# NeuralRevenant/RASSEngine

Hardware: NVIDIA B200
Metric: exact top-10 QPS @10M x 1024 (cosine, ids identical to the fp64 CPU oracle) (higher is better)
Workload: dtype bf16 scan (fp32 accumulate) + fp64 rerank

## Files before the change

rassengine_b200/csrc/common.cuh:

```cuda
#pragma once
#include <cuda_runtime.h>
#include <cuda_bf16.h>
#include <stdint.h>
#include <stdio.h>
#include <string>
#include <vector>

#include "../../include/rass_b200.h"

#define RASS_WARPS_PER_CTA 8
#define RASS_MAX_K 128
#define RASS_CAND_MAX 2048
#define RASS_GROUP_Q 64
#define RASS_QPAD 256
#define RASS_STREAM_SEG 64
static inline int rass_tc_seg(int k) { return k > 32 ? 512 : 256; }
__host__ __device__ constexpr int rass_tc_keep(int seg) { return seg == 512 ? 128 : seg / 8; }
#define RASS_EXACT_NQ 4
#define RASS_FINISH_THREADS 1024

struct RowMap {
  int64_t base;
  int32_t g, G, blk_log2;
};
#define RASS_SHARD_BLOCK_LOG2 10
__host__ __device__ inline int64_t row_local_to_global(const RowMap& m, int64_t local) {
  if (m.G <= 1) return m.base + local;
  const int64_t b = local >> m.blk_log2, in = local & ((int64_t(1) << m.blk_log2) - 1);
  return m.base + (((b * m.G + m.g) << m.blk_log2) | in);
}
__host__ __device__ inline int64_t row_global_to_local(const RowMap& m, int64_t global) {
  const int64_t r = global - m.base;
  if (r < 0) return -1;
  if (m.G <= 1) return r;
  const int64_t b = r >> m.blk_log2;
  if ((int32_t)(b % m.G) != m.g) return -1;
  return ((b / m.G) << m.blk_log2) | (r & ((int64_t(1) << m.blk_log2) - 1));
}

#define HYB_TILE 4096
#define HYB_TABLE_MIN_DF 512

struct TextSegment {
  int field = 0;
  int64_t n_post = 0, n_uniq = 0;
  int32_t* uterm = nullptr;
  int64_t* uptr = nullptr;
  int32_t* doc = nullptr;
  uint16_t* tf = nullptr;
};

struct Bm25State {
  bool built = false;
  int64_t V = 0, N = 0, nnz = 0;
  int F = 1;
  std::vector<uint8_t> term_field_host;
  int64_t* indptr = nullptr;
  int32_t* doc = nullptr;
  uint16_t* tf = nullptr;
  float* xq = nullptr;
  uint8_t* norm = nullptr;
  float* inv_dev = nullptr;
  int n_tiles = 0;
  uint32_t* tile_off = nullptr;
  std::vector<int32_t> table_row_host;
  unsigned char* qt_host = nullptr;
  unsigned char* qt_dev = nullptr;
  size_t qt_cap = 0, qt_q_cap = 0, qt_bytes = 0;
  uint32_t* hyb_gthr = nullptr;
  uint32_t* vocab_blob = nullptr;
  int64_t* vocab_off = nullptr;
  int64_t vocab_V = 0;
  int32_t* fz_terms = nullptr;
  int32_t* fz_edits = nullptr;
  int* fz_n = nullptr;
  float avgdl = 0.f;
  int64_t doc_count = 0;
  std::vector<int64_t> indptr_host;
  std::vector<float> idf_host;
  std::vector<float> xmin_host, xmax_host;
  bool force_ordered = false;
  bool maxscore = false;
  int* sel_fallback = nullptr;
  std::vector<TextSegment> pending;
  uint32_t* doclen_dev = nullptr;
  uint32_t* gen_dev = nullptr;
  bool has_rewrite = false;
  int doclen_F = 0;
  int64_t doclen_stride = 0;
  std::vector<int64_t> field_vocab;
  std::vector<int64_t> field_last_row;
  bool contiguous_fields = true;
  std::vector<int64_t> field_doc_count, field_sum_ttf;
  std::vector<uint8_t> field_omit_norms;
  int64_t pending_V = 0;
  void* scratch = nullptr;
  size_t scratch_bytes = 0;
};

struct StoreScalars {
  float rho_x;
  float max_xnorm;
  float rho_x8;
};

struct SearchScalars {
  int flagged_n;
  int max_cand;
  int n_certified;
  int finish_done;
  int tile_ctr[2];
};

struct SearchWs {
  SearchScalars* scal = nullptr;
  int q_cap = 0;
  float* q_raw = nullptr;
  float* q_hat = nullptr;
  __nv_bfloat16* q16 = nullptr;
  double* q_norm = nullptr;
  float* q_rho = nullptr;
  int8_t* q8 = nullptr;
  float* q8_scale = nullptr;
  float* q_rho8 = nullptr;
  uint32_t* q_gthr = nullptr;
  size_t pool_entries = 0;
  size_t pool_alloc_entries = 0;
  float* pool_key = nullptr;
  uint32_t* pool_row = nullptr;
  size_t pool_segs = 0;
  size_t pool_alloc_segs = 0;
  float* pool_thr = nullptr;
  int* pool_cnt = nullptr;
  int* flagged = nullptr;
  int* flagged_host = nullptr;
  void* tmap_q = nullptr;
  void* tmap_q2 = nullptr;
  const void* tmap_qbase = nullptr;
  const void* tmap_q2base = nullptr;
  void* tmap_q8 = nullptr;
  const void* tmap_q8base = nullptr;
};

struct VmArray {
  void* base = nullptr;
  size_t reserved = 0, mapped = 0, chunk = 0;
  int device = 0;
  std::vector<unsigned long long> handles;
};
bool vm_available();
bool vm_reserve(VmArray* a, int device, size_t max_bytes, size_t chunk_hint);
int vm_grow(VmArray* a, size_t bytes);
void vm_free(VmArray* a);

struct rass_engine {
  int dim = 0, dim_pad = 0, metric = 0, device = 0;
  uint32_t flags = 0;
  int num_sms = 0;
  int path = RASS_PATH_AUTO;
  int64_t cap = 0, n_rows = 0, n_live = 0;
  RowMap rmap = {0, 0, 1, RASS_SHARD_BLOCK_LOG2};
  struct ShardSet* shards = nullptr;
  float* x32 = nullptr;
  __nv_bfloat16* x16 = nullptr;
  double* norm64 = nullptr;
  float* sa = nullptr;
  float* sb = nullptr;
  int8_t* x8 = nullptr;
  float* sa8 = nullptr;
  VmArray vm[7];
  bool use_vm = false;
  StoreScalars* store_scal = nullptr;
  StoreScalars store_scal_host = {};
  bool store_scal_stale = false;
  int int8_k_max = RASS_MAX_K;
  SearchWs ws[2];
  SearchScalars* scal_host = nullptr;
  cudaStream_t stream = nullptr, user_stream = nullptr, copy_stream = nullptr;
  bool has_user_stream = false;
  cudaEvent_t ev[4] = {nullptr, nullptr, nullptr, nullptr};
  cudaEvent_t stage_ev[2] = {nullptr, nullptr};
  float* stage[2] = {nullptr, nullptr};
  size_t stage_bytes = 0;
  float* dev_stage = nullptr;
  size_t dev_stage_bytes = 0;
  size_t xlist_entries = 0;
  double* xlist_key = nullptr;
  uint32_t* xlist_row = nullptr;
  int64_t* out_rows = nullptr;
  float* out_scores = nullptr;
  double* out_keys = nullptr;
  size_t out_cap = 0;
  int64_t* out_rows_host = nullptr;
  float* out_scores_host = nullptr;
  double* out_keys_host = nullptr;
  float* q_stage_host = nullptr;
  float* q_stage_dev = nullptr;
  size_t q_stage_cap = 0;
  std::vector<uint8_t> dead;
  std::vector<cudaEvent_t> ev_pool;
  void* tmap_x = nullptr;
  int64_t tmap_rows = -1;
  const void* tmap_base = nullptr;
  void* tmap_x8 = nullptr;
  int64_t tmap8_rows = -1;
  const void* tmap8_base = nullptr;
  int* retry_ids = nullptr;
  float* retry_q = nullptr;
  int64_t* retry_rows = nullptr;
  float* retry_scores = nullptr;
  double* retry_keys = nullptr;
  size_t retry_cap = 0;
  int retry_k = 0;
  bool async_overlap = false;
  int scan_reserve_sms = 0;
  cudaStream_t slot_stream[2] = {nullptr, nullptr};
  cudaEvent_t slot_fork[2] = {nullptr, nullptr};
  struct AsyncSlot {
    bool pending = false, trivial = false;
    int k = 0;
    SearchScalars* scal_host = nullptr;
    cudaEvent_t done = nullptr;
    size_t n_ev = 0;
    rass_stats stats;
  } aslot[2];
  int64_t* flist_dev = nullptr;
  size_t flist_cap = 0;
  uint8_t* row_filter = nullptr;
  int64_t* filter_rows_dev = nullptr;
  size_t filter_rows_cap = 0;
  bool knn_prefilter = false;
  float* sb_filtered = nullptr;
  int64_t sb_filtered_cap = 0;
  bool sb_filtered_dirty = true;
  const float* sb_scan = nullptr;
  int64_t row_filter_rows = 0;
  size_t row_filter_cap = 0;
  Bm25State bm25;
  rass_stats last_stats = {};
  std::string err;
};

extern thread_local std::string g_create_error;

int rass_fail(rass_engine* h, int code, const char* fmt, ...);

#define CUDA_TRY(h, call)                                                                         \
  do {                                                                                            \
    cudaError_t e_ = (call);                                                                      \
    if (e_ != cudaSuccess)                                                                        \
      return rass_fail((h), e_ == cudaErrorMemoryAllocation ? RASS_E_OOM : RASS_E_CUDA,           \
                       "%s failed: %s (%s:%d)", #call, cudaGetErrorString(e_), __FILE__, __LINE__); \
  } while (0)

static inline cudaStream_t eng_stream(const rass_engine* h) { return h->has_user_stream ? h->user_stream : h->stream; }
static inline cudaStream_t slot_stream_of(const rass_engine* h, int slot) {
  return h->async_overlap && h->slot_stream[slot] ? h->slot_stream[slot] : eng_stream(h);
}

static inline float acc_allowance(int dim_pad) { return (float)dim_pad * 1.1920929e-7f; }

static inline bool has_int8_shadow(uint32_t flags) { return !(flags & (RASS_BF16_ONLY | RASS_NO_INT8_SHADOW)); }

#ifdef __CUDACC__

__device__ __forceinline__ uint4 ldg_stream(const uint4* p) {
  uint4 r;
  asm volatile("ld.global.nc.L1::no_allocate.v4.u32 {%0, %1, %2, %3}, [%4];"
               : "=r"(r.x), "=r"(r.y), "=r"(r.z), "=r"(r.w)
               : "l"(p));
  return r;
}

__device__ __forceinline__ float bf16lo(uint32_t p) { return __uint_as_float(p << 16); }
__device__ __forceinline__ float bf16hi(uint32_t p) { return __uint_as_float(p & 0xffff0000u); }

template <typename K>
__device__ __forceinline__ K neg_inf();
template <>
__device__ __forceinline__ float neg_inf<float>() { return __int_as_float(0xff800000); }
template <>
__device__ __forceinline__ double neg_inf<double>() { return __longlong_as_double(0xfff0000000000000ULL); }

template <typename K>
__device__ __forceinline__ bool entry_better(K ka, uint32_t ra, K kb, uint32_t rb) {
  return ka > kb || (ka == kb && ra < rb);
}

__device__ __forceinline__ float shfl_xor_t(float v, int m) { return __shfl_xor_sync(0xffffffffu, v, m); }
__device__ __forceinline__ double shfl_xor_t(double v, int m) { return __shfl_xor_sync(0xffffffffu, v, m); }
__device__ __forceinline__ float shfl_t(float v, int l) { return __shfl_sync(0xffffffffu, v, l); }
__device__ __forceinline__ double shfl_t(double v, int l) { return __shfl_sync(0xffffffffu, v, l); }

__device__ __forceinline__ double warp_sum(double v) {
#pragma unroll
  for (int m = 16; m >= 1; m >>= 1) v += __shfl_xor_sync(0xffffffffu, v, m);
  return v;
}

__device__ __forceinline__ uint32_t ord32(float f) {
  const uint32_t u = __float_as_uint(f);
  return (u & 0x80000000u) ? ~u : (u | 0x80000000u);
}
__device__ __forceinline__ float unord32(uint32_t o) {
  return __uint_as_float((o & 0x80000000u) ? (o & 0x7fffffffu) : ~o);
}

template <int E>
__device__ __forceinline__ int warp_compact(const uint32_t (&ok)[E], const uint32_t (&rw)[E], int keep,
                                            float* out_key, uint32_t* out_row, uint32_t& pivot) {
  const int lane = threadIdx.x & 31;
  uint32_t kmin = 0xffffffffu, kmax = 0;
#pragma unroll
  for (int i = 0; i < E; ++i)
    if (ok[i]) { kmin = min(kmin, ok[i]); kmax = max(kmax, ok[i]); }
  kmin = __reduce_min_sync(0xffffffffu, kmin);
  kmax = __reduce_max_sync(0xffffffffu, kmax);
  uint32_t lo = kmin - 1, hi = kmax;
  pivot = kmax;
  int total = 0;
#pragma unroll
  for (int i = 0; i < E; ++i) total += ok[i] != 0;
  total = __reduce_add_sync(0xffffffffu, total);
  if (total <= 2 * keep) {
    pivot = 0x007fffffu;
  } else {
    bool found = false;
    while (hi - lo > 1) {
      const uint32_t mid = lo + ((hi - lo) >> 1);
      int cgt = 0;
#pragma unroll
      for (int i = 0; i < E; ++i) cgt += ok[i] > mid;
      cgt = __reduce_add_sync(0xffffffffu, cgt);
      if (cgt > 2 * keep) lo = mid;
      else if (cgt < keep) hi = mid;
      else { pivot = mid; found = true; break; }
    }
    if (!found) pivot = hi;
  }
  int kept = 0;
#pragma unroll
  for (int i = 0; i < E; ++i) {
    const bool k = ok[i] > pivot;
    const unsigned bal = __ballot_sync(0xffffffffu, k);
    if (k) {
      const int pos = kept + __popc(bal & ((1u << lane) - 1));
      out_key[pos] = unord32(ok[i]);
      out_row[pos] = rw[i];
    }
    kept += __popc(bal);
  }
  return kept;
}

template <typename K, int M>
struct WarpTop {
  K key[M];
  uint32_t row[M];
  K thr_key;
  uint32_t thr_row;

  __device__ __forceinline__ void init() {
#pragma unroll
    for (int i = 0; i < M; ++i) { key[i] = neg_inf<K>(); row[i] = 0xffffffffu; }
    thr_key = neg_inf<K>();
    thr_row = 0xffffffffu;
  }

  __device__ __forceinline__ bool admits_ascending(K k) const { return k > thr_key; }

  __device__ __noinline__ void insert(K k, uint32_t r) {
    if (!entry_better<K>(k, r, thr_key, thr_row)) return;
    const int lane = threadIdx.x & 31;
    int slot = -1;
#pragma unroll
    for (int i = M - 1; i >= 0; --i)
      if (key[i] == thr_key && row[i] == thr_row) slot = i;
    unsigned holders = __ballot_sync(0xffffffffu, slot >= 0);
    int owner = __ffs(holders) - 1;
    if (lane == owner) {
#pragma unroll
      for (int i = 0; i < M; ++i)
        if (i == slot) { key[i] = k; row[i] = r; }
    }
    K wk = key[0];
    uint32_t wr = row[0];
#pragma unroll
    for (int i = 1; i < M; ++i)
      if (entry_better<K>(wk, wr, key[i], row[i])) { wk = key[i]; wr = row[i]; }
#pragma unroll
    for (int m = 16; m >= 1; m >>= 1) {
      K ok = shfl_xor_t(wk, m);
      uint32_t orow = __shfl_xor_sync(0xffffffffu, wr, m);
      if (entry_better<K>(wk, wr, ok, orow)) { wk = ok; wr = orow; }
    }
    thr_key = wk;
    thr_row = wr;
  }
};

template <bool BF16_ROWS>
__device__ __forceinline__ double exact_key_warp(const float* __restrict__ x32, const __nv_bfloat16* __restrict__ x16,
                                                 const double* __restrict__ norm64, uint32_t row, const float* qs,
                                                 double qnorm, int dim_pad, int metric) {
  const int lane = threadIdx.x & 31;
  double acc = 0.0;
  if (BF16_ROWS) {
    const uint4* p = reinterpret_cast<const uint4*>(x16 + (size_t)row * dim_pad);
    for (int j = lane; j < dim_pad / 8; j += 32) {
      uint4 v = __ldg(p + j);
      const uint32_t w[4] = {v.x, v.y, v.z, v.w};
      const float* qq = qs + j * 8;
#pragma unroll
      for (int e = 0; e < 4; ++e) {
        double a = (double)bf16lo(w[e]), b = (double)bf16hi(w[e]);
        double q0 = (double)qq[2 * e], q1 = (double)qq[2 * e + 1];
        if (metric == RASS_METRIC_COSINE) {
          acc = fma(a, q0, acc);
          acc = fma(b, q1, acc);
        } else {
          double d0 = a - q0, d1 = b - q1;
          acc = fma(d0, d0, acc);
          acc = fma(d1, d1, acc);
        }
      }
    }
  } else {
    const float4* p = reinterpret_cast<const float4*>(x32 + (size_t)row * dim_pad);
    for (int j = lane; j < dim_pad / 4; j += 32) {
      float4 v = __ldg(p + j);
      const float4 q = *reinterpret_cast<const float4*>(qs + j * 4);
      if (metric == RASS_METRIC_COSINE) {
        acc = fma((double)v.x, (double)q.x, acc);
        acc = fma((double)v.y, (double)q.y, acc);
        acc = fma((double)v.z, (double)q.z, acc);
        acc = fma((double)v.w, (double)q.w, acc);
      } else {
        double d0 = (double)v.x - (double)q.x, d1 = (double)v.y - (double)q.y;
        double d2 = (double)v.z - (double)q.z, d3 = (double)v.w - (double)q.w;
        acc = fma(d0, d0, acc);
        acc = fma(d1, d1, acc);
        acc = fma(d2, d2, acc);
        acc = fma(d3, d3, acc);
      }
    }
  }
  acc = warp_sum(acc);
  if (metric == RASS_METRIC_COSINE) {
    double den = norm64[row] * qnorm;
    return den > 0.0 ? acc / den : 0.0;
  }
  return -acc;
}

__device__ __forceinline__ float int8_key(int32_t acc1, int32_t acc2, float s1, float s2, float sa8, float sb) {
  return __fmaf_rn(__fmaf_rn(s1, __int2float_rn(acc1), __fmul_rn(s2, __int2float_rn(acc2))), sa8, sb);
}

__device__ __forceinline__ float warp_max_nonneg(float v) {
  return __uint_as_float(__reduce_max_sync(0xffffffffu, __float_as_uint(v)));
}

__device__ __forceinline__ float int8_code(float v, float s) {
  return s > 0.f ? fminf(fmaxf(rintf(__fdiv_rn(v, s)), -127.f), 127.f) : 0.f;
}

__device__ __forceinline__ float score_from_key(double key, int metric) {
  return metric == RASS_METRIC_COSINE ? (float)(1.0 / (2.0 - key)) : (float)(1.0 / (1.0 - key));
}

#endif

int launch_store_convert(rass_engine* h, const float* src_dev, int64_t src_stride, int64_t first_row, int64_t n,
                         cudaStream_t st);
int launch_query_prep(rass_engine* h, const SearchWs& ws, const float* q_dev, int B, cudaStream_t st);
int launch_seed_thresholds(rass_engine* h, const SearchWs& ws, int B, int seg, size_t n_clear, bool* cleared,
                           cudaStream_t st, bool int8 = false);
int launch_scan_stream(rass_engine* h, const SearchWs& ws, int q0, int nq, int g0, cudaStream_t st);
int scan_stream_segs(const rass_engine* h);
int launch_scan_umma(rass_engine* h, SearchWs& ws, int q0, int nq, int seg, cudaStream_t st, bool pool_cleared = false,
                     bool int8 = false);
int scan_umma_segs(const rass_engine* h);
int umma_selftest(rass_engine* h, SearchWs& ws, int n_rows_tile, float* out_host, cudaStream_t st);
int umma8_selftest(rass_engine* h, SearchWs& ws, int32_t* out_host, cudaStream_t st);
int launch_scan_gemm(rass_engine* h, SearchWs& ws, int B, int seg, cudaStream_t st, bool pool_cleared = false);
int scan_gemm_segs(const rass_engine* h, int B);
int gemm_selftest(rass_engine* h, SearchWs& ws, int B, float* out_host, cudaStream_t st);
int encode_rows_map(rass_engine* h, void* map, const void* base, int64_t rows, int box_rows, int elem_bytes = 2);
enum ScanOperands { SCAN_FP32_Q = 0, SCAN_BF16 = 1, SCAN_INT8 = 2 };
int launch_finish(rass_engine* h, const SearchWs& ws, int g0, int ng, int k, int n_segs, int seg_size, bool has_cnt,
                  ScanOperands ops, int64_t* out_rows, float* out_scores, double* out_keys, cudaStream_t st,
                  int64_t* flag_out = nullptr);
int launch_exact(rass_engine* h, const SearchWs& ws, int k, const int* qids_host, int n_q, int64_t* out_rows,
                 float* out_scores, double* out_keys, cudaStream_t st, int* launches);
int launch_merge_topk(rass_engine* h, const double* keys, const int64_t* rows, int64_t shard_stride, int G, int B,
                      int k, int64_t* out_rows, float* out_scores, double* out_keys, cudaStream_t st,
                      bool raw_score = false);
int search_core(rass_engine* h, const float* q_dev, int B, int k, int64_t* out_rows, float* out_scores,
                double* out_keys, rass_stats* stats, int async_slot = -1, int64_t* async_flag_dev = nullptr);
int stage_queries(rass_engine* h, const float* q_host, int B, float** q_dev_out);
struct HybridExt {
  const int64_t* knn_rows_dev;
  const float* knn_scores_dev;
  int64_t* out_rows_dev;
  float* out_scores_dev;
  double* out_keys_dev;
};
struct HybridTerms {
  const int32_t* qt_indptr;
  const int64_t* t_lo;
  const uint32_t* t_len;
  const float* t_w;
  const int32_t* t_row;
  const float* t_bound;
  const uint8_t* t_field;
  const uint8_t* t_flag;
  bool multi, order_free;
  size_t n_terms;
  int64_t postings;
};
typedef HybridTerms FilteredTermArrays;
int stage_hybrid_terms(rass_engine* h, int B, const int32_t* qterm_indptr, const int32_t* qterms, const float* qweights,
                       const uint8_t* qflags, float w_text, HybridTerms* out, cudaStream_t st);
int hybrid_core(rass_engine* h, const float* q_host, int B, const int32_t* qterm_indptr, const int32_t* qterms,
                const float* qweights, const uint8_t* qflags, float w_text, float w_knn, int k, int64_t* out_rows,
                float* out_scores, rass_stats* stats, const HybridExt* ext = nullptr);
int bm25_build_impl(rass_engine* h, const int64_t* indptr, const int32_t* doc, const uint16_t* tf,
                    const int32_t* term_field, const uint32_t* doclen, int64_t V, int64_t N, int F,
                    const int64_t* g_doc_count, const int64_t* g_sum_ttf, const int64_t* g_df);
int sharded_destroy(rass_engine* h);
int sharded_set_option(rass_engine* h, int opt, int64_t value);
int sharded_set_row_base(rass_engine* h, int64_t base);
int sharded_sync(rass_engine* h);
int sharded_append(rass_engine* h, const float* rows_host, int64_t n, int64_t* out_first_row);
int sharded_append_dev(rass_engine* h, const float* rows_dev, int64_t n, int64_t* out_first_row);
int sharded_overwrite(rass_engine* h, int64_t row, const float* v_host);
int sharded_tombstone(rass_engine* h, int64_t row);
int sharded_read_rows(rass_engine* h, int64_t first_row, int64_t n, float* out_host);
int sharded_read_rows_list(rass_engine* h, const int64_t* rows_host, int64_t n, float* out_host);
int sharded_set_row_filter(rass_engine* h, const uint8_t* mask_host, int64_t n);
int sharded_set_row_filter_rows(rass_engine* h, const int64_t* rows_host, int64_t n, int64_t total_rows);
int sharded_search_knn(rass_engine* h, const float* q_host, int B, int k, int64_t* out_rows, float* out_scores,
                       double* out_keys, rass_stats* stats);
int sharded_search_knn_dev(rass_engine* h, const float* q_dev, int B, int k, int64_t* out_rows_dev,
                           float* out_scores_dev, double* out_keys_dev, rass_stats* stats);
int sharded_search_knn_dev_async(rass_engine* h, const float* q_dev, int B, int k, int64_t* out_rows_dev,
                                 float* out_scores_dev, double* out_keys_dev, int slot, int64_t* flag_out_dev);
int sharded_search_knn_dev_wait(rass_engine* h, int slot, rass_stats* stats);
int sharded_async_join(rass_engine* h, int slot, void* stream);
int sharded_bm25_build(rass_engine* h, const int64_t* indptr, const int32_t* doc, const uint16_t* tf,
                       const int32_t* term_field, const uint32_t* doclen, int64_t V, int64_t N, int F);
int sharded_search_hybrid(rass_engine* h, const float* q_host, int B, const int32_t* qterm_indptr, const int32_t* qterms,
                          const float* qweights, const uint8_t* qflags, float w_text, float w_knn, int k,
                          int64_t* out_rows, float* out_scores, rass_stats* stats);
int sharded_fuse_hybrid(rass_engine* h, int B, const int32_t* qterm_indptr, const int32_t* qterms,
                        const float* qweights, const uint8_t* qflags, float w_text, const int64_t* knn_rows_host,
                        const float* knn_scores_host, float w_knn, int k, int64_t* out_rows, float* out_scores);
int sharded_save(rass_engine* h, const char* path);
int sharded_text_add_rows(rass_engine* h, int field, const int64_t* rows, int64_t n_rows, const int64_t* tok_indptr,
                          const int32_t* tok_terms);
int sharded_text_commit(rass_engine* h, const int64_t* field_vocab, int F, int64_t N);
int sharded_text_size(rass_engine* h, int64_t* V, int64_t* N, int64_t* nnz, int* F);
int sharded_text_stats(rass_engine* h, int64_t* indptr, int64_t* doc_count, int64_t* sum_ttf);
int text_commit_merge(rass_engine* h, const int64_t* field_vocab, int F, int64_t N);
int text_local_stats(rass_engine* h, int F, int64_t N, int64_t* doc_count, int64_t* sum_ttf);
int text_finalize_global(rass_engine* h, int64_t N, int F, const int64_t* g_doc_count, const int64_t* g_sum_ttf,
                         const int64_t* global_df);
const std::vector<rass_engine*>& sharded_shards(rass_engine* h);
rass_engine* sharded_first(rass_engine* h);
#define SHARDED(h, call)                 \
  do {                                   \
    if ((h) && (h)->shards) return call; \
  } while (0)

int ensure_query_workspace(rass_engine* h, SearchWs& ws, int B);
int ensure_pool(rass_engine* h, SearchWs& ws, size_t entries_per_query, size_t segs_per_query,
                size_t n_queries = RASS_GROUP_Q);
int ensure_xlist_workspace(rass_engine* h, size_t entries);
int ensure_out_workspace(rass_engine* h, size_t n);
```

rassengine_b200/csrc/finish.cu:

```cuda
#include "common.cuh"

struct FinishArgs {
  const float* pool_key;
  const uint32_t* pool_row;
  const float* pool_thr;
  const int* pool_cnt;
  size_t pool_entries;
  int n_segs, seg_size;
  const float* x32;
  const __nv_bfloat16* x16;
  const double* norm64;
  const float* q_raw;
  const double* q_norm;
  const float* q_rho;
  const StoreScalars* store;
  int int8;
  SearchScalars* scal;
  int* flagged;
  int dim_pad, metric, k, g0;
  float acc_eps;
  RowMap rmap;
  int64_t* out_rows;
  float* out_scores;
  double* out_keys;
  int64_t* flag_out;
};

template <bool BF16_ROWS>
__global__ void __launch_bounds__(RASS_FINISH_THREADS, 1) finish_kernel(FinishArgs a) {
  extern __shared__ __align__(16) unsigned char smem_raw[];
  float* qs = reinterpret_cast<float*>(smem_raw);
  double* ckey = reinterpret_cast<double*>(qs + a.dim_pad);
  uint32_t* crow = reinterpret_cast<uint32_t*>(ckey + RASS_CAND_MAX);
  __shared__ float s_red[32];
  __shared__ int s_redi[32];
  __shared__ float s_t;
  __shared__ int s_valid, s_ncand, s_have;
  __shared__ double s_sk;

  const int tid = threadIdx.x, lane = tid & 31, warp = tid >> 5;
  const int slot = blockIdx.x;
  const int q = a.g0 + slot;
  const float* pk = a.pool_key + (size_t)slot * a.pool_entries;
  const uint32_t* pr = a.pool_row + (size_t)slot * a.pool_entries;

  for (int j = tid; j < a.dim_pad; j += blockDim.x) qs[j] = a.q_raw[(size_t)q * a.dim_pad + j];
  if (tid == 0) { s_ncand = 0; s_have = 0; }

  float mx = neg_inf<float>();
  int nvalid = 0;
  for (int sgm = warp; sgm < a.n_segs; sgm += RASS_FINISH_THREADS / 32) {
    const int cnt = a.pool_cnt ? min(a.pool_cnt[(size_t)slot * a.n_segs + sgm], a.seg_size) : a.seg_size;
    for (int i = lane; i < cnt; i += 32) {
      const size_t o = (size_t)sgm * a.seg_size + i;
      if (a.pool_cnt || pr[o] != 0xffffffffu) {
        ++nvalid;
        mx = fmaxf(mx, pk[o]);
      }
    }
  }
  float t = neg_inf<float>();
  for (int s = tid; s < a.n_segs; s += blockDim.x) t = fmaxf(t, a.pool_thr[(size_t)slot * a.n_segs + s]);
#pragma unroll
  for (int m = 16; m >= 1; m >>= 1) {
    t = fmaxf(t, __shfl_xor_sync(0xffffffffu, t, m));
    nvalid += __shfl_xor_sync(0xffffffffu, nvalid, m);
  }
  if (lane == 0) { s_red[warp] = t; s_redi[warp] = nvalid; }
  __syncthreads();
  if (warp == 0) {
    float tt = s_red[lane];
    int nv = s_redi[lane];
#pragma unroll
    for (int m = 16; m >= 1; m >>= 1) {
      tt = fmaxf(tt, __shfl_xor_sync(0xffffffffu, tt, m));
      nv += __shfl_xor_sync(0xffffffffu, nv, m);
    }
    if (lane == 0) { s_t = tt; s_valid = nv; }
  }

  float bprime;
  {
    const uint32_t mine = mx > neg_inf<float>() ? ord32(mx) : 0u;
    uint32_t prefix = 0;
#pragma unroll 1
    for (int bit = 31; bit >= 0; --bit) {
      const uint32_t cand = prefix | (1u << bit);
      if (__syncthreads_count(mine >= cand) >= a.k) prefix = cand;
    }
    bprime = prefix > 0x007fffffu ? unord32(prefix) : neg_inf<float>();
  }

  float eps;
  {
    const float rho_x = a.int8 ? a.store->rho_x8 : (BF16_ROWS ? 0.f : a.store->rho_x);
    const float rho_q = a.q_rho ? a.q_rho[q] : 0.f;
    float e = rho_x * (1.f + rho_q) + rho_q + a.acc_eps;
    if (a.metric == RASS_METRIC_L2) {
      const float xm = a.store->max_xnorm;
      e = e * xm * (float)a.q_norm[q] * 1.0001f + 6.0e-8f * xm * xm;
    }
    eps = e * 1.0001f;
  }
  const float cutoff = bprime - 2.f * eps;

  for (int sgm = warp; sgm < a.n_segs; sgm += RASS_FINISH_THREADS / 32) {
    const int cnt = a.pool_cnt ? min(a.pool_cnt[(size_t)slot * a.n_segs + sgm], a.seg_size) : a.seg_size;
    for (int i = lane; i < cnt; i += 32) {
      const size_t o = (size_t)sgm * a.seg_size + i;
      if ((a.pool_cnt || pr[o] != 0xffffffffu) && pk[o] >= cutoff) {
        int pos = atomicAdd(&s_ncand, 1);
        if (pos < RASS_CAND_MAX) crow[pos] = pr[o];
      }
    }
  }
  __syncthreads();
  const int ncand_raw = s_ncand;
  const int ncand = min(ncand_raw, RASS_CAND_MAX);

  const double qn = a.q_norm[q];
  for (int c = warp; c < ncand; c += RASS_FINISH_THREADS / 32) {
    double key = exact_key_warp<BF16_ROWS>(a.x32, a.x16, a.norm64, crow[c], qs, qn, a.dim_pad, a.metric);
    if (lane == 0) ckey[c] = key;
  }
  __syncthreads();

  const int kk = a.k;
  for (int c = tid; c < ncand; c += blockDim.x) {
    const double key = ckey[c];
    const uint32_t row = crow[c];
    int rank = 0;
    for (int j = 0; j < ncand; ++j) rank += entry_better<double>(ckey[j], crow[j], key, row);
    if (rank < kk) {
      const size_t o = (size_t)q * kk + rank;
      a.out_rows[o] = row_local_to_global(a.rmap, (int64_t)row);
      a.out_scores[o] = score_from_key(key, a.metric);
      if (a.out_keys) a.out_keys[o] = a.metric == RASS_METRIC_COSINE ? key : -key;
      if (rank == kk - 1) { s_sk = key; s_have = 1; }
    }
  }
  for (int r = ncand + tid; r < kk; r += blockDim.x) {
    const size_t o = (size_t)q * kk + r;
    a.out_rows[o] = -1;
    a.out_scores[o] = 0.f;
    if (a.out_keys) a.out_keys[o] = 0.0;
  }
  __syncthreads();

  if (tid == 0) {
    bool ok;
    const float tt = s_t;
    if (ncand_raw > RASS_CAND_MAX) {
      ok = false;
    } else if (!s_have) {
      ok = (tt == neg_inf<float>()) && ncand == s_valid;
    } else if (tt == neg_inf<float>()) {
      ok = true;
    } else {
      double sk = s_sk;
      if (a.metric == RASS_METRIC_L2) sk = 0.5 * (qn * qn + sk);
      ok = (double)tt + (double)eps < sk;
    }
    if (ok) {
      atomicAdd(&a.scal->n_certified, 1);
    } else {
      int pos = atomicAdd(&a.scal->flagged_n, 1);
      a.flagged[pos] = q;
    }
    atomicMax(&a.scal->max_cand, ncand_raw);
    if (a.flag_out) {
      __threadfence();
      if (atomicAdd(&a.scal->finish_done, 1) == (int)gridDim.x - 1) {
        a.scal->finish_done = 0;
        *a.flag_out = (int64_t)atomicAdd(&a.scal->flagged_n, 0);
      }
    }
  }
}

static size_t finish_smem(int dim_pad) {
  return (size_t)dim_pad * 4 + RASS_CAND_MAX * 12;
}

int launch_finish(rass_engine* h, const SearchWs& ws, int g0, int ng, int k, int n_segs, int seg_size, bool has_cnt,
                  ScanOperands ops, int64_t* out_rows, float* out_scores, double* out_keys, cudaStream_t st,
                  int64_t* flag_out) {
  FinishArgs a;
  a.flag_out = flag_out;
  a.pool_key = ws.pool_key;
  a.pool_row = ws.pool_row;
  a.pool_thr = ws.pool_thr;
  a.pool_cnt = has_cnt ? ws.pool_cnt : nullptr;
  a.pool_entries = ws.pool_entries;
  a.n_segs = n_segs;
  a.seg_size = seg_size;
  a.x32 = h->x32;
  a.x16 = h->x16;
  a.norm64 = h->norm64;
  a.q_raw = ws.q_raw;
  a.q_norm = ws.q_norm;
  a.q_rho = ops == SCAN_INT8 ? ws.q_rho8 : (ops == SCAN_BF16 ? ws.q_rho : nullptr);
  a.int8 = ops == SCAN_INT8;
  a.store = h->store_scal;
  a.scal = ws.scal;
  a.flagged = ws.flagged;
  a.dim_pad = h->dim_pad;
  a.metric = h->metric;
  a.k = k;
  a.g0 = g0;
  a.acc_eps = acc_allowance(h->dim_pad);
  a.rmap = h->rmap;
  a.out_rows = out_rows;
  a.out_scores = out_scores;
  a.out_keys = out_keys;
  const size_t smem = finish_smem(h->dim_pad);
  if (h->flags & RASS_BF16_ONLY) {
    CUDA_TRY(h, cudaFuncSetAttribute(finish_kernel<true>, cudaFuncAttributeMaxDynamicSharedMemorySize, (int)smem));
    finish_kernel<true><<<ng, RASS_FINISH_THREADS, smem, st>>>(a);
  } else {
    CUDA_TRY(h, cudaFuncSetAttribute(finish_kernel<false>, cudaFuncAttributeMaxDynamicSharedMemorySize, (int)smem));
    finish_kernel<false><<<ng, RASS_FINISH_THREADS, smem, st>>>(a);
  }
  CUDA_TRY(h, cudaGetLastError());
  return RASS_OK;
}

template <bool BF16_ROWS, int M>
__global__ void __launch_bounds__(RASS_WARPS_PER_CTA * 32) exact_scan_kernel(
    const float* __restrict__ x32, const __nv_bfloat16* __restrict__ x16, const double* __restrict__ norm64,
    const float* __restrict__ sb, const float* __restrict__ q_raw, const double* __restrict__ q_norm,
    const int* __restrict__ qids, int nq, int64_t n_rows, int dim_pad, int metric, double* __restrict__ xkey,
    uint32_t* __restrict__ xrow, size_t xlist_entries) {
  extern __shared__ __align__(16) unsigned char smem_raw[];
  float* qs = reinterpret_cast<float*>(smem_raw);
  const int lane = threadIdx.x & 31, warp = threadIdx.x >> 5;
  const int gw = blockIdx.x * RASS_WARPS_PER_CTA + warp;
  const int W = gridDim.x * RASS_WARPS_PER_CTA;
  for (int i = threadIdx.x; i < nq * dim_pad; i += blockDim.x)
    qs[i] = q_raw[(size_t)qids[i / dim_pad] * dim_pad + (i % dim_pad)];
  __syncthreads();
  double qn[RASS_EXACT_NQ];
  WarpTop<double, M> top[RASS_EXACT_NQ];
#pragma unroll
  for (int i = 0; i < RASS_EXACT_NQ; ++i) {
    top[i].init();
    qn[i] = i < nq ? q_norm[qids[i]] : 0.0;
  }
  for (int64_t row = gw; row < n_rows; row += W) {
    if (sb[row] == neg_inf<float>()) continue;
#pragma unroll
    for (int i = 0; i < RASS_EXACT_NQ; ++i) {
      if (i < nq) {
        double key = exact_key_warp<BF16_ROWS>(x32, x16, norm64, (uint32_t)row, qs + (size_t)i * dim_pad, qn[i],
                                               dim_pad, metric);
        if (top[i].admits_ascending(key)) top[i].insert(key, (uint32_t)row);
      }
    }
  }
#pragma unroll
  for (int i = 0; i < RASS_EXACT_NQ; ++i) {
    if (i < nq) {
      const size_t base = (size_t)i * xlist_entries + (size_t)gw * (32 * M);
#pragma unroll
      for (int s = 0; s < M; ++s) {
        xkey[base + s * 32 + lane] = top[i].key[s];
        xrow[base + s * 32 + lane] = top[i].row[s];
      }
    }
  }
}

__device__ __forceinline__ uint64_t ord64(double d) {
  if (d == 0.0) d = 0.0;
  uint64_t u = (uint64_t)__double_as_longlong(d);
  return (u >> 63) ? ~u : (u | 0x8000000000000000ULL);
}

__global__ void __launch_bounds__(1024, 1) exact_select_kernel(const double* __restrict__ xkey,
                                                               const uint32_t* __restrict__ xrow, size_t xlist_entries,
                                                               int n, int k, const int* __restrict__ qids, int q_fixed,
                                                               int raw_score, int metric,
                                                               RowMap rmap, int64_t* __restrict__ out_rows,
                                                               float* __restrict__ out_scores,
                                                               double* __restrict__ out_keys,
                                                               const int* __restrict__ only_if) {
  if (only_if && !only_if[blockIdx.x]) return;
  __shared__ int hist[256];
  __shared__ int s_bucket, s_remaining, s_nsel, s_nvalid;
  __shared__ double selk[RASS_MAX_K];
  __shared__ uint32_t selr[RASS_MAX_K];
  const int tid = threadIdx.x;
  const int q = qids ? qids[blockIdx.x] : q_fixed + (int)blockIdx.x;
  const double* key = xkey + (size_t)blockIdx.x * xlist_entries;
  const uint32_t* row = xrow + (size_t)blockIdx.x * xlist_entries;

  if (tid == 0) { s_nvalid = 0; s_nsel = 0; }
  __syncthreads();
  int nv = 0;
  for (int i = tid; i < n; i += blockDim.x) nv += row[i] != 0xffffffffu;
  if (nv) atomicAdd(&s_nvalid, nv);
  __syncthreads();
  const int kk = min(k, s_nvalid);

  uint64_t pre_hi = 0, mask_hi = 0;
  uint32_t pre_lo = 0, mask_lo = 0;
  if (kk > 0) {
    if (tid == 0) s_remaining = kk;
    for (int byte = 11; byte >= 0; --byte) {
      for (int b = tid; b < 256; b += blockDim.x) hist[b] = 0;
      __syncthreads();
      for (int i = tid; i < n; i += blockDim.x) {
        const uint32_t r = row[i];
        if (r == 0xffffffffu) continue;
        const uint64_t hi = ord64(key[i]);
        const uint32_t lo = ~r;
        if ((hi & mask_hi) != pre_hi || (lo & mask_lo) != pre_lo) continue;
        const int b = byte >= 4 ? (int)((hi >> ((byte - 4) * 8)) & 255) : (int)((lo >> (byte * 8)) & 255);
        atomicAdd(&hist[b], 1);
      }
      __syncthreads();
      if (tid < 32) {
        int loc[8], sum = 0;
#pragma unroll
        for (int i = 0; i < 8; ++i) { loc[i] = hist[8 * tid + i]; sum += loc[i]; }
        int suf = sum;
#pragma unroll
        for (int m = 1; m < 32; m <<= 1) {
          const int o = __shfl_down_sync(0xffffffffu, suf, m);
          if (tid + m < 32) suf += o;
        }
        const int rem = s_remaining, above = suf - sum;
        if (above < rem && rem <= above + sum) {
          int cum = above;
#pragma unroll
          for (int i = 7; i >= 0; --i) {
            if (cum + loc[i] >= rem) { s_bucket = 8 * tid + i; s_remaining = rem - cum; break; }
            cum += loc[i];
          }
        }
      }
      __syncthreads();
      const int b = s_bucket;
      if (byte >= 4) {
        pre_hi |= (uint64_t)b << ((byte - 4) * 8);
        mask_hi |= (uint64_t)255 << ((byte - 4) * 8);
      } else {
        pre_lo |= (uint32_t)b << (byte * 8);
        mask_lo |= (uint32_t)255 << (byte * 8);
      }
      __syncthreads();
    }
    for (int i = tid; i < n; i += blockDim.x) {
      const uint32_t r = row[i];
      if (r == 0xffffffffu) continue;
      const uint64_t hi = ord64(key[i]);
      const uint32_t lo = ~r;
      if (hi > pre_hi || (hi == pre_hi && lo >= pre_lo)) {
        int pos = atomicAdd(&s_nsel, 1);
        if (pos < RASS_MAX_K) { selk[pos] = key[i]; selr[pos] = r; }
      }
    }
  }
  __syncthreads();
  const int nsel = min(s_nsel, RASS_MAX_K);
  for (int c = tid; c < nsel; c += blockDim.x) {
    int rank = 0;
    for (int j = 0; j < nsel; ++j) rank += entry_better<double>(selk[j], selr[j], selk[c], selr[c]);
    if (rank < k) {
      const size_t o = (size_t)q * k + rank;
      out_rows[o] = row_local_to_global(rmap, (int64_t)selr[c]);
      out_scores[o] = raw_score ? (float)selk[c] : score_from_key(selk[c], metric);
      if (out_keys) out_keys[o] = metric == RASS_METRIC_COSINE ? selk[c] : -selk[c];
    }
  }
  for (int r = nsel + tid; r < k; r += blockDim.x) {
    const size_t o = (size_t)q * k + r;
    out_rows[o] = -1;
    out_scores[o] = 0.f;
    if (out_keys) out_keys[o] = 0.0;
  }
}

int launch_exact(rass_engine* h, const SearchWs& ws, int k, const int* qids_host, int n_q, int64_t* out_rows,
                 float* out_scores, double* out_keys, cudaStream_t st, int* launches) {
  if (n_q <= 0) return RASS_OK;
  const int M = k <= 32 ? 1 : 4;
  const int grid = h->num_sms * 2;
  const int W = grid * RASS_WARPS_PER_CTA;
  const size_t entries = (size_t)W * 32 * M;
  int rc = ensure_xlist_workspace(h, entries);
  if (rc) return rc;
  const bool bf = (h->flags & RASS_BF16_ONLY) != 0;
  const size_t smem = (size_t)RASS_EXACT_NQ * h->dim_pad * 4;
  int* qids_dev = ws.flagged;
  CUDA_TRY(h, cudaMemcpyAsync(qids_dev, qids_host, (size_t)n_q * sizeof(int), cudaMemcpyHostToDevice, st));
  for (int p = 0; p < n_q; p += RASS_EXACT_NQ) {
    const int nq = n_q - p < RASS_EXACT_NQ ? n_q - p : RASS_EXACT_NQ;
#define RASS_EX(BF, MM)                                                                                           \
  exact_scan_kernel<BF, MM><<<grid, RASS_WARPS_PER_CTA * 32, smem, st>>>(                                         \
      h->x32, h->x16, h->norm64, h->sb_scan, ws.q_raw, ws.q_norm, qids_dev + p, nq, h->n_rows, h->dim_pad, h->metric, \
      h->xlist_key, h->xlist_row, entries)
    if (bf) { if (M == 1) RASS_EX(true, 1); else RASS_EX(true, 4); }
    else    { if (M == 1) RASS_EX(false, 1); else RASS_EX(false, 4); }
#undef RASS_EX
    CUDA_TRY(h, cudaGetLastError());
    exact_select_kernel<<<nq, 1024, 0, st>>>(h->xlist_key, h->xlist_row, entries, (int)entries, k, qids_dev + p, 0, 0,
                                             h->metric, h->rmap, out_rows, out_scores, out_keys, nullptr);
    CUDA_TRY(h, cudaGetLastError());
    if (launches) *launches += 2;
  }
  return RASS_OK;
}

int launch_exact_select(rass_engine* h, size_t entries, int B, int k, int64_t* out_rows, float* out_scores,
                        double* out_keys, cudaStream_t st) {
  exact_select_kernel<<<B, 1024, 0, st>>>(h->xlist_key, h->xlist_row, entries, (int)entries, k, nullptr, 0, 0, h->metric,
                                          h->rmap, out_rows, out_scores, out_keys, nullptr);
  CUDA_TRY(h, cudaGetLastError());
  return RASS_OK;
}

int launch_select_batch(rass_engine* h, size_t entries, int B, int k, int64_t* out_rows, float* out_scores,
                        double* out_keys, cudaStream_t st, const int* only_if) {
  exact_select_kernel<<<B, 1024, 0, st>>>(h->xlist_key, h->xlist_row, entries, (int)entries, k, nullptr, 0, 1,
                                          RASS_METRIC_COSINE, h->rmap, out_rows, out_scores, out_keys, only_if);
  CUDA_TRY(h, cudaGetLastError());
  return RASS_OK;
}

__global__ void __launch_bounds__(256) merge_topk_kernel(const double* __restrict__ keys,
                                                         const int64_t* __restrict__ rows, int64_t shard_stride,
                                                         int G, int B, int k,
                                                         int metric, int raw_score, int64_t* __restrict__ out_rows,
                                                         float* __restrict__ out_scores,
                                                         double* __restrict__ out_keys) {
  extern __shared__ __align__(16) unsigned char smem_raw[];
  double* sk = reinterpret_cast<double*>(smem_raw);
  int64_t* sr = reinterpret_cast<int64_t*>(sk + G * k);
  const int q = blockIdx.x, n = G * k;
  for (int i = threadIdx.x; i < n; i += blockDim.x) {
    const int g = i / k, j = i % k;
    const size_t src = (size_t)g * shard_stride + (size_t)q * k + j;
    const double v = keys[src];
    sk[i] = (raw_score || metric == RASS_METRIC_COSINE) ? v : -v;
    sr[i] = rows[src];
  }
  __syncthreads();
  int n_valid = 0;
  for (int i = threadIdx.x; i < n; i += blockDim.x) {
    const int64_t r = sr[i];
    if (r < 0) continue;
    const double key = sk[i];
    int rank = 0;
    for (int j = 0; j < n; ++j) {
      const int64_t rj = sr[j];
      if (rj < 0) continue;
      rank += (sk[j] > key) || (sk[j] == key && rj < r);
    }
    if (rank < k) {
      const size_t o = (size_t)q * k + rank;
      out_rows[o] = r;
      out_scores[o] = raw_score ? (float)key : score_from_key(key, metric);
      if (out_keys) out_keys[o] = (raw_score || metric == RASS_METRIC_COSINE) ? key : -key;
    }
  }
  for (int j = 0; j < n; ++j) n_valid += sr[j] >= 0;
  for (int r = n_valid + threadIdx.x; r < k; r += blockDim.x) {
    const size_t o = (size_t)q * k + r;
    out_rows[o] = -1;
    out_scores[o] = 0.f;
    if (out_keys) out_keys[o] = 0.0;
  }
}

int launch_merge_topk(rass_engine* h, const double* keys, const int64_t* rows, int64_t shard_stride, int G, int B,
                      int k, int64_t* out_rows, float* out_scores, double* out_keys, cudaStream_t st, bool raw_score) {
  if (shard_stride <= 0) shard_stride = (int64_t)B * k;
  const size_t smem = (size_t)G * k * 16;
  if (smem > 200 * 1024) return rass_fail(h, RASS_E_INVALID, "merge of %d lists of %d exceeds shared memory", G, k);
  CUDA_TRY(h, cudaFuncSetAttribute(merge_topk_kernel, cudaFuncAttributeMaxDynamicSharedMemorySize, (int)smem));
  merge_topk_kernel<<<B, 256, smem, st>>>(keys, rows, shard_stride, G, B, k, h->metric, raw_score ? 1 : 0, out_rows,
                                          out_scores, out_keys);
  CUDA_TRY(h, cudaGetLastError());
  return RASS_OK;
}
```

Baseline: 35220.

## Bitonic-sort rerank candidates, specialize exact key by dim, batch pool scans

Replaces the O(n^2) rank-counting selection in the finish kernel with a shared-memory bitonic sort over candidates padded to a power of two. It also specializes the fp64 exact-key computation on dim_pad and metric so the row loads are fully unrolled and issued up front. Pool scans now batch eight loads per lane, prefetch the next segment count, and skip row loads when they are not needed. The sort adds many __syncthreads passes, and the unrolled loads raise register pressure in a 1024-thread kernel.

```diff
diff --git a/rassengine_b200/csrc/common.cuh b/rassengine_b200/csrc/common.cuh
--- a/rassengine_b200/csrc/common.cuh
+++ b/rassengine_b200/csrc/common.cuh
@@ -399,58 +399,68 @@
   }
 };
 
+template <bool COSINE>
+__device__ __forceinline__ double key_term(double acc, double x, double q) {
+  if (COSINE) return fma(x, q, acc);
+  const double d = x - q;
+  return fma(d, d, acc);
+}
+
+template <bool BF16_ROWS, bool COSINE, int NV>
+__device__ __forceinline__ double row_lane_sum(const uint4 (&v)[NV], const float* qs, int lane) {
+  double acc = 0.0;
+#pragma unroll
+  for (int i = 0; i < NV; ++i) {
+    const int j = lane + 32 * i;
+    const uint32_t w[4] = {v[i].x, v[i].y, v[i].z, v[i].w};
+    if (BF16_ROWS) {
+      const float* qq = qs + j * 8;
+#pragma unroll
+      for (int e = 0; e < 4; ++e) {
+        acc = key_term<COSINE>(acc, (double)bf16lo(w[e]), (double)qq[2 * e]);
+        acc = key_term<COSINE>(acc, (double)bf16hi(w[e]), (double)qq[2 * e + 1]);
+      }
+    } else {
+      const float4 q = *reinterpret_cast<const float4*>(qs + j * 4);
+      acc = key_term<COSINE>(acc, (double)__uint_as_float(w[0]), (double)q.x);
+      acc = key_term<COSINE>(acc, (double)__uint_as_float(w[1]), (double)q.y);
+      acc = key_term<COSINE>(acc, (double)__uint_as_float(w[2]), (double)q.z);
+      acc = key_term<COSINE>(acc, (double)__uint_as_float(w[3]), (double)q.w);
+    }
+  }
+  return acc;
+}
+
+template <bool BF16_ROWS, int DIM_PAD>
+__device__ __forceinline__ double exact_key_warp_dp(const float* __restrict__ x32, const __nv_bfloat16* __restrict__ x16,
+                                                    const double* __restrict__ norm64, uint32_t row, const float* qs,
+                                                    double qnorm, int metric) {
+  constexpr int NV = DIM_PAD / (BF16_ROWS ? 256 : 128);
+  const int lane = threadIdx.x & 31;
+  const uint4* p = BF16_ROWS ? reinterpret_cast<const uint4*>(x16 + (size_t)row * DIM_PAD)
+                             : reinterpret_cast<const uint4*>(x32 + (size_t)row * DIM_PAD);
+  uint4 v[NV];
+#pragma unroll
+  for (int i = 0; i < NV; ++i) v[i] = __ldg(p + lane + 32 * i);
+  if (metric == RASS_METRIC_COSINE) {
+    const double xn = __ldg(norm64 + row);
+    const double acc = warp_sum(row_lane_sum<BF16_ROWS, true>(v, qs, lane));
+    const double den = xn * qnorm;
+    return den > 0.0 ? acc / den : 0.0;
+  }
+  return -warp_sum(row_lane_sum<BF16_ROWS, false>(v, qs, lane));
+}
+
 template <bool BF16_ROWS>
 __device__ __forceinline__ double exact_key_warp(const float* __restrict__ x32, const __nv_bfloat16* __restrict__ x16,
                                                  const double* __restrict__ norm64, uint32_t row, const float* qs,
                                                  double qnorm, int dim_pad, int metric) {
-  const int lane = threadIdx.x & 31;
-  double acc = 0.0;
-  if (BF16_ROWS) {
-    const uint4* p = reinterpret_cast<const uint4*>(x16 + (size_t)row * dim_pad);
-    for (int j = lane; j < dim_pad / 8; j += 32) {
-      uint4 v = __ldg(p + j);
-      const uint32_t w[4] = {v.x, v.y, v.z, v.w};
-      const float* qq = qs + j * 8;
-#pragma unroll
-      for (int e = 0; e < 4; ++e) {
-        double a = (double)bf16lo(w[e]), b = (double)bf16hi(w[e]);
-        double q0 = (double)qq[2 * e], q1 = (double)qq[2 * e + 1];
-        if (metric == RASS_METRIC_COSINE) {
-          acc = fma(a, q0, acc);
-          acc = fma(b, q1, acc);
-        } else {
-          double d0 = a - q0, d1 = b - q1;
-          acc = fma(d0, d0, acc);
-          acc = fma(d1, d1, acc);
-        }
-      }
-    }
-  } else {
-    const float4* p = reinterpret_cast<const float4*>(x32 + (size_t)row * dim_pad);
-    for (int j = lane; j < dim_pad / 4; j += 32) {
-      float4 v = __ldg(p + j);
-      const float4 q = *reinterpret_cast<const float4*>(qs + j * 4);
-      if (metric == RASS_METRIC_COSINE) {
-        acc = fma((double)v.x, (double)q.x, acc);
-        acc = fma((double)v.y, (double)q.y, acc);
-        acc = fma((double)v.z, (double)q.z, acc);
-        acc = fma((double)v.w, (double)q.w, acc);
-      } else {
-        double d0 = (double)v.x - (double)q.x, d1 = (double)v.y - (double)q.y;
-        double d2 = (double)v.z - (double)q.z, d3 = (double)v.w - (double)q.w;
-        acc = fma(d0, d0, acc);
-        acc = fma(d1, d1, acc);
-        acc = fma(d2, d2, acc);
-        acc = fma(d3, d3, acc);
-      }
-    }
-  }
-  acc = warp_sum(acc);
-  if (metric == RASS_METRIC_COSINE) {
-    double den = norm64[row] * qnorm;
-    return den > 0.0 ? acc / den : 0.0;
-  }
-  return -acc;
+  switch (dim_pad) {
+    case 256: return exact_key_warp_dp<BF16_ROWS, 256>(x32, x16, norm64, row, qs, qnorm, metric);
+    case 512: return exact_key_warp_dp<BF16_ROWS, 512>(x32, x16, norm64, row, qs, qnorm, metric);
+    case 768: return exact_key_warp_dp<BF16_ROWS, 768>(x32, x16, norm64, row, qs, qnorm, metric);
+    default: return exact_key_warp_dp<BF16_ROWS, 1024>(x32, x16, norm64, row, qs, qnorm, metric);
+  }
 }
 
 __device__ __forceinline__ float int8_key(int32_t acc1, int32_t acc2, float s1, float s2, float sa8, float sb) {
diff --git a/rassengine_b200/csrc/finish.cu b/rassengine_b200/csrc/finish.cu
--- a/rassengine_b200/csrc/finish.cu
+++ b/rassengine_b200/csrc/finish.cu
@@ -26,6 +26,9 @@
   int64_t* flag_out;
 };
 
+#define RASS_FINISH_BATCH 8
+static_assert((RASS_CAND_MAX & (RASS_CAND_MAX - 1)) == 0, "the rerank sort pads the candidates to a power of two");
+
 template <bool BF16_ROWS>
 __global__ void __launch_bounds__(RASS_FINISH_THREADS, 1) finish_kernel(FinishArgs a) {
   extern __shared__ __align__(16) unsigned char smem_raw[];
@@ -35,9 +38,9 @@
   __shared__ float s_red[32];
   __shared__ int s_redi[32];
   __shared__ float s_t;
-  __shared__ int s_valid, s_ncand, s_have;
-  __shared__ double s_sk;
-
+  __shared__ int s_valid, s_ncand;
+
+  constexpr int NW = RASS_FINISH_THREADS / 32;
   const int tid = threadIdx.x, lane = tid & 31, warp = tid >> 5;
   const int slot = blockIdx.x;
   const int q = a.g0 + slot;
@@ -45,20 +48,41 @@
   const uint32_t* pr = a.pool_row + (size_t)slot * a.pool_entries;
 
   for (int j = tid; j < a.dim_pad; j += blockDim.x) qs[j] = a.q_raw[(size_t)q * a.dim_pad + j];
-  if (tid == 0) { s_ncand = 0; s_have = 0; }
+  if (tid == 0) s_ncand = 0;
+
+  auto seg_count = [&](int sgm) {
+    if (sgm >= a.n_segs) return 0;
+    return a.pool_cnt ? min(__ldg(a.pool_cnt + (size_t)slot * a.n_segs + sgm), a.seg_size) : a.seg_size;
+  };
+  auto for_each_entry = [&](bool need_rows, auto&& visit) {
+    const bool load_rows = need_rows || !a.pool_cnt;
+    int cnt_next = seg_count(warp);
+    for (int sgm = warp; sgm < a.n_segs; sgm += NW) {
+      const int cnt = cnt_next;
+      cnt_next = seg_count(sgm + NW);
+      const size_t base = (size_t)sgm * a.seg_size;
+      for (int i0 = 0; i0 < cnt; i0 += 32 * RASS_FINISH_BATCH) {
+        float kv[RASS_FINISH_BATCH];
+        uint32_t rv[RASS_FINISH_BATCH];
+#pragma unroll
+        for (int u = 0; u < RASS_FINISH_BATCH; ++u) {
+          const int i = i0 + 32 * u + lane;
+          kv[u] = i < cnt ? __ldg(pk + base + i) : 0.f;
+          rv[u] = i < cnt && load_rows ? __ldg(pr + base + i) : 0xffffffffu;
+        }
+#pragma unroll
+        for (int u = 0; u < RASS_FINISH_BATCH; ++u)
+          if (i0 + 32 * u + lane < cnt && (a.pool_cnt || rv[u] != 0xffffffffu)) visit(kv[u], rv[u]);
+      }
+    }
+  };
 
   float mx = neg_inf<float>();
   int nvalid = 0;
-  for (int sgm = warp; sgm < a.n_segs; sgm += RASS_FINISH_THREADS / 32) {
-    const int cnt = a.pool_cnt ? min(a.pool_cnt[(size_t)slot * a.n_segs + sgm], a.seg_size) : a.seg_size;
-    for (int i = lane; i < cnt; i += 32) {
-      const size_t o = (size_t)sgm * a.seg_size + i;
-      if (a.pool_cnt || pr[o] != 0xffffffffu) {
-        ++nvalid;
-        mx = fmaxf(mx, pk[o]);
-      }
-    }
-  }
+  for_each_entry(false, [&](float key, uint32_t) {
+    ++nvalid;
+    mx = fmaxf(mx, key);
+  });
   float t = neg_inf<float>();
   for (int s = tid; s < a.n_segs; s += blockDim.x) t = fmaxf(t, a.pool_thr[(size_t)slot * a.n_segs + s]);
 #pragma unroll
@@ -104,60 +128,71 @@
   }
   const float cutoff = bprime - 2.f * eps;
 
-  for (int sgm = warp; sgm < a.n_segs; sgm += RASS_FINISH_THREADS / 32) {
-    const int cnt = a.pool_cnt ? min(a.pool_cnt[(size_t)slot * a.n_segs + sgm], a.seg_size) : a.seg_size;
-    for (int i = lane; i < cnt; i += 32) {
-      const size_t o = (size_t)sgm * a.seg_size + i;
-      if ((a.pool_cnt || pr[o] != 0xffffffffu) && pk[o] >= cutoff) {
-        int pos = atomicAdd(&s_ncand, 1);
-        if (pos < RASS_CAND_MAX) crow[pos] = pr[o];
-      }
-    }
-  }
+  for_each_entry(true, [&](float key, uint32_t row) {
+    if (key >= cutoff) {
+      const int pos = atomicAdd(&s_ncand, 1);
+      if (pos < RASS_CAND_MAX) crow[pos] = row;
+    }
+  });
   __syncthreads();
   const int ncand_raw = s_ncand;
   const int ncand = min(ncand_raw, RASS_CAND_MAX);
+  int npad = 1;
+  while (npad < ncand) npad <<= 1;
 
   const double qn = a.q_norm[q];
-  for (int c = warp; c < ncand; c += RASS_FINISH_THREADS / 32) {
+  for (int c = warp; c < ncand; c += NW) {
     double key = exact_key_warp<BF16_ROWS>(a.x32, a.x16, a.norm64, crow[c], qs, qn, a.dim_pad, a.metric);
     if (lane == 0) ckey[c] = key;
   }
-  __syncthreads();
+  for (int c = ncand + tid; c < npad; c += blockDim.x) {
+    ckey[c] = neg_inf<double>();
+    crow[c] = 0xffffffffu;
+  }
+  __syncthreads();
+
+  for (int size = 2; size <= npad; size <<= 1) {
+    for (int stride = size >> 1; stride > 0; stride >>= 1) {
+      for (int i = tid; i < npad / 2; i += blockDim.x) {
+        const int lo = 2 * i - (i & (stride - 1)), hi = lo + stride;
+        const double klo = ckey[lo], khi = ckey[hi];
+        const uint32_t rlo = crow[lo], rhi = crow[hi];
+        const bool best_first = (lo & size) == 0;
+        if (best_first ? entry_better<double>(khi, rhi, klo, rlo) : entry_better<double>(klo, rlo, khi, rhi)) {
+          ckey[lo] = khi; ckey[hi] = klo;
+          crow[lo] = rhi; crow[hi] = rlo;
+        }
+      }
+      __syncthreads();
+    }
+  }
 
   const int kk = a.k;
-  for (int c = tid; c < ncand; c += blockDim.x) {
-    const double key = ckey[c];
-    const uint32_t row = crow[c];
-    int rank = 0;
-    for (int j = 0; j < ncand; ++j) rank += entry_better<double>(ckey[j], crow[j], key, row);
-    if (rank < kk) {
-      const size_t o = (size_t)q * kk + rank;
-      a.out_rows[o] = row_local_to_global(a.rmap, (int64_t)row);
+  for (int r = tid; r < kk; r += blockDim.x) {
+    const size_t o = (size_t)q * kk + r;
+    if (r < ncand) {
+      const double key = ckey[r];
+      a.out_rows[o] = row_local_to_global(a.rmap, (int64_t)crow[r]);
       a.out_scores[o] = score_from_key(key, a.metric);
       if (a.out_keys) a.out_keys[o] = a.metric == RASS_METRIC_COSINE ? key : -key;
-      if (rank == kk - 1) { s_sk = key; s_have = 1; }
-    }
-  }
-  for (int r = ncand + tid; r < kk; r += blockDim.x) {
-    const size_t o = (size_t)q * kk + r;
-    a.out_rows[o] = -1;
-    a.out_scores[o] = 0.f;
-    if (a.out_keys) a.out_keys[o] = 0.0;
-  }
-  __syncthreads();
+    } else {
+      a.out_rows[o] = -1;
+      a.out_scores[o] = 0.f;
+      if (a.out_keys) a.out_keys[o] = 0.0;
+    }
+  }
 
   if (tid == 0) {
     bool ok;
     const float tt = s_t;
     if (ncand_raw > RASS_CAND_MAX) {
       ok = false;
-    } else if (!s_have) {
+    } else if (ncand < kk) {
       ok = (tt == neg_inf<float>()) && ncand == s_valid;
     } else if (tt == neg_inf<float>()) {
       ok = true;
     } else {
-      double sk = s_sk;
+      double sk = ckey[kk - 1];
       if (a.metric == RASS_METRIC_L2) sk = 0.5 * (qn * qn + sk);
       ok = (double)tt + (double)eps < sk;
     }
```

Measured after the change: 35940, median of 6. +2.0%, better.
